# atakan-topaloglu/stable-virtual-camera

Hardware: AMD Instinct MI355X
Metric: denoising steps/sec, 1.3B Seva @ 21x576x576 views (higher is better)
Workload: dtype f16; 1 GPU; Seva 1.3B (1,263,968,004 params, random-init), one 21-view window per GPU, 576x576 px (latent 72x72), CFG batch 42, Euler-EDM step, MultiviewCFG(1.2) cfg 2.0; novel_views_per_sec = value x (T - 1 input view) / 50 steps per window; views=21, latent=72, windows=1

## Files before the change

### include/seva_hip.h

```cpp
#ifndef SEVA_HIP_H
#define SEVA_HIP_H

#include <stdint.h>

#ifdef __cplusplus
extern "C" {
#endif

typedef void* seva_stream_t;

#define SEVA_OK 0
#define SEVA_ERR_ARG (-1)
#define SEVA_ERR_LAUNCH (-2)
#define SEVA_ERR_UNSUPPORTED (-3)

const char* seva_last_error(void);
int seva_abi_version(void);
const char* seva_target_arch(void);

typedef struct seva_gemm_desc {
  const void* a;
  const void* w;
  const float* bias;
  const float* row_add;
// ... 14 lines not shown
  void* out_f8;
  int64_t ldo8;
  float* ch_stats;
  float* splitk_ws;
  int64_t splitk_ws_bytes;
  const void* a2;
  int64_t lda2;
  int64_t K2;
  int64_t alg_K;
} seva_gemm_desc;
int seva_gemm_f16(const seva_gemm_desc* d, seva_stream_t stream);
int seva_gemm_fp8(const seva_gemm_desc* d, seva_stream_t stream);

typedef struct seva_ff_desc {
  const void* a;
  const void* w1;
  const float* b1;
  const void* w2;
  const float* b2;
  const float* residual;
  float* out_f32;
  void* out_f16;
  int64_t M, lda, ldr, ldo32, ldo16;
  int32_t C;
  const float* ln_x;
  const float* ln_gamma;
  const float* ln_beta;
  int64_t ldx;
  float ln_eps;
  const void* w1_exp;
  const void* w2_exp;
} seva_ff_desc;
int seva_ff_fused_f16(const seva_ff_desc* d, seva_stream_t stream);
int seva_ff_fused_fp8(const seva_ff_desc* d, seva_stream_t stream);

typedef struct seva_attn_desc {
  const void* q;
  const void* k;
  const void* v;
  void* out;
  int64_t q_sb0, q_sb1, q_sl;
  int64_t k_sb0, k_sb1, k_sl;
  int64_t o_sb0, o_sb1, o_sl;
  int32_t nb0, nb1;
  int32_t heads;
  int32_t lq, lk;
  float scale;
  int32_t q_prescaled;
  float* split_ws;
  int64_t split_ws_bytes;
} seva_attn_desc;
int seva_attention_f16(const seva_attn_desc* d, seva_stream_t stream);

int seva_attn_v_fp8_size(int32_t batch, int32_t heads, int32_t lk, int64_t* v8_bytes, int64_t* scale_bytes);
int seva_attn_quant_v_fp8(const seva_attn_desc* d, void* v8, uint8_t* v8_scale, seva_stream_t stream);
int seva_attention_pv8(const seva_attn_desc* d, const void* v8, const uint8_t* v8_scale, seva_stream_t stream);

#define SEVA_GN_WORKSPACE_SLABS 1024
typedef struct seva_groupnorm_desc {
  const float* x1;
  const float* x2;
  const float* gamma;
  const float* beta;
  const float* dense;
  const float* dense_w;
  const float* dense_b;
  void* out_f16;
  float* workspace;
  int32_t n, hw, c1, c2, groups, dense_c, silu;
  float eps;
  void* raw_f16;
  void* out_f8;
  int64_t ld_out_f8;
  const float* stats1;
  const float* stats2;
  int32_t split_out_f16;
  int32_t split_raw_f16;
} seva_groupnorm_desc;
int seva_groupnorm_f16(const seva_groupnorm_desc* d, seva_stream_t stream);

int seva_layernorm_f16(const float* x, const float* gamma, const float* beta, void* out_f16,
                       int64_t rows, int32_t c, float eps, seva_stream_t stream);
int seva_layernorm_fp8(const float* x, const float* gamma, const float* beta, void* out_f8, int64_t rows,
                       int32_t c, float eps, int64_t ld_out ,
                       seva_stream_t stream);

int seva_softmax_rows_f16(const float* x, int64_t ldx, void* out_f16, int64_t ldo, int64_t rows,
                          int32_t cols, int32_t cols_pad, float scale, seva_stream_t stream);

int seva_nchw_to_nhwc_f16(const float* x1, int32_t c1, const float* x2, int32_t c2,
                          const float* scale, void* out_f16, int32_t n, int32_t hw, int32_t cpad,
                          seva_stream_t stream);
int seva_nchw_to_nhwc_f16_split(const float* x1, int32_t c1, const float* x2, int32_t c2,
                                const float* scale, void* out_f16, int32_t n, int32_t hw, int32_t cpad,
                                seva_stream_t stream);
int seva_nhwc_to_nchw_f32(const float* x, int64_t ld, float* out, int32_t n, int32_t c,
                          int32_t hw, seva_stream_t stream);
int seva_cast_concat_f16(const float* x1, int32_t c1, const float* x2, int32_t c2, void* out_f16,
                         int64_t rows, seva_stream_t stream);
int seva_bilinear_to_nhwc_f32(const float* src, float* out, int32_t n, int32_t c, int32_t sh,
                              int32_t sw, int32_t oh, int32_t ow, seva_stream_t stream);
int seva_timestep_embedding_f16(const int64_t* t, const float* freqs, void* out_f16, int32_t n,
                                int32_t dim, seva_stream_t stream);
int seva_silu_f16(const float* x, void* out_f16, int64_t count, seva_stream_t stream);
int seva_add_f32(const float* a, const float* b, float* out, int64_t count, seva_stream_t stream);

// ... 51 lines not shown
```

### stable-virtual-camera_amd/seva/_engine.py

```python

from __future__ import annotations

import math
import os

import torch

from . import _native, ops
from ._arch import Layout
from ._native import SevaNativeError, require_cuda

F16, F32, U8 = torch.float16, torch.float32, torch.uint8
QK_SCALE_LOG2E = 0.125 * 1.4426950408889634
CIN_PAD = 64


def _pad128(k: int) -> int:
    return 128 * ((k + 127) // 128)


def pack_conv3x3(w: torch.Tensor, cin_pad: int | None = None) -> torch.Tensor:
    cout, cin = w.shape[:2]
    cin_pad = cin_pad or cin
    out = torch.zeros((cout, 3, 3, cin_pad), dtype=F16, device=w.device)
# ... 38 lines not shown

    def nbytes(self) -> int:
        return sum(t.numel() * t.element_size() for t in self.bufs.values())


class SevaEngine:
    @staticmethod
    def _resolve_device(model) -> torch.device:
        params = [p for p in model.parameters()]
        if not params or params[0].device.type != "cuda":
            raise SevaNativeError(
                "Seva.forward runs only on an AMD GPU: move the module to a cuda device first "
                "(there is no CPU fallback)."
            )
        from . import _native

        _native.load()
        return params[0].device

    def __init__(self, model, precision: str | None = None, attention: str | None = None, ff: str | None = None):
        import os as _os

        self.device = self._resolve_device(model)
        self.precision = precision or _os.environ.get("SEVA_PRECISION", "f16")
        if self.precision not in ("f16", "fp8"):
            raise ValueError(f"unknown precision {self.precision!r} (f16 | fp8)")
        self.fp8 = self.precision == "fp8"
        if attention is None:
            attention = "fp8" if self.fp8 and _os.environ.get("SEVA_FP8_ATTENTION", "0") == "1" else "f16"
        if attention not in ("f16", "fp8"):
            raise ValueError(f"unknown attention {attention!r} (f16 | fp8)")
        if attention == "fp8" and not self.fp8:
            raise ValueError('attention="fp8" needs precision "fp8" (the f16 parity mode stays pure)')
        self.attention = attention
        self.pv8 = attention == "fp8"
        self.fp8_pad = _os.environ.get("SEVA_FP8_PAD", "0") == "1"
        self.ff_fused = _os.environ.get("SEVA_FF_FUSED", "1") != "0"
        if ff is None:
            ff = "fp8" if self.fp8 and _os.environ.get("SEVA_FP8_FF", "0") == "1" else "f16"
        if ff not in ("f16", "fp8"):
            raise ValueError(f"unknown ff {ff!r} (f16 | fp8)")
        if ff == "fp8" and not self.fp8:
            raise ValueError('ff="fp8" needs precision "fp8" (the f16 parity mode stays pure)')
        self.ff = ff
        self.ff8 = ff == "fp8"
        self.gn_fused_stats = int(_os.environ.get("SEVA_GN_FUSED_STATS", "1"))
        self._stats: dict = {}
        self.conv_splitk = _os.environ.get("SEVA_CONV_SPLITK", "1") != "0"
        self.attn_split = _os.environ.get("SEVA_ATTN_SPLIT_KV", "1") != "0"
        self.attn_split_max = max(2, min(4, int(_os.environ.get("SEVA_ATTN_SPLIT", "2"))))
        self.fold_skip = _os.environ.get("SEVA_FOLD_SKIP", "0") != "0" and not self.fp8
        sp = _os.environ.get("SEVA_SPLIT_PRECISION", "stem,head,skip_deep")
        self.split = {t for t in sp.split(",") if t} if not self.fp8 else set()
        self.p = model.params
        self.layout: Layout = model._layout
        self.arena = _Arena(self.device)
        self._pack(model)
        import os

        self.use_graph = os.environ.get("SEVA_HIPGRAPH", "1") != "0"
        self._graphs: dict = {}
        self.slice_frames = int(os.environ.get("SEVA_SLICE_FRAMES", "0"))
        self.slice_min_bytes = int(float(os.environ.get("SEVA_SLICE_MIN_MB", "96")) * (1 << 20))
        self.slice_attn = os.environ.get("SEVA_SLICE_ATTN", "0") == "1"

    def _ff_fused_fp8(self, c: int) -> bool:
        return self.ff8 and self.ff_fused and c in ops.FF_FUSED_CHANNELS and c % 128 != 0

    def _split_skip(self, cout: int) -> bool:
        return "skip" in self.split or ("skip_deep" in self.split and cout >= 2 * self.p.model_channels)

    def _pack(self, model) -> None:
        sd = {k: v.detach() for k, v in model.state_dict().items()}
        dev = self.device
        W: dict[str, torch.Tensor] = {}

        def f16(k):
            return sd[k].to(device=dev, dtype=F16).contiguous()

        def f32(k):
            return sd[k].to(device=dev, dtype=F32).contiguous()

        mc = self.p.model_channels
        half = mc // 2
        W["freqs"] = torch.exp(
            -math.log(10000) * torch.arange(start=0, end=half, dtype=torch.float32) / half
        ).to(dev)
        for k in ("time_embed.0", "time_embed.2"):
            W[k + ".w"], W[k + ".b"] = f16(k + ".weight"), f32(k + ".bias")

        emb_w, emb_b, ctx_w, ctx_b = [], [], [], []
        self.emb_off: dict[str, int] = {}
        self.ctx_off: dict[str, int] = {}
        emb_total = ctx_total = 0

        def q8(name, w):
            if not (self.fp8 and w.shape[0] % 16 == 0 and w.shape[0] > 32):
                return
            k = w.shape[1]
            kp = _pad128(k)
            if kp != k and (not self.fp8_pad or kp * 4 > k * 5):
                return
            if kp != k:
                w = torch.cat([w, w.new_zeros((w.shape[0], kp - k))], 1)
            W[name + "8"], W[name + "8e"] = ops.quantize_weight_fp8(w)

        def pack_attn_self(pfx):
            W[pfx + ".qkv"] = torch.cat(
                [f16(pfx + ".to_q.weight"), f16(pfx + ".to_k.weight"), f16(pfx + ".to_v.weight")], 0
            ).contiguous()
            q8(pfx + ".qkv", torch.cat([f32(pfx + ".to_q.weight"), f32(pfx + ".to_k.weight"), f32(pfx + ".to_v.weight")], 0))
            W[pfx + ".out.w"], W[pfx + ".out.b"] = f16(pfx + ".to_out.0.weight"), f32(pfx + ".to_out.0.bias")

        def pack_attn_cross(pfx):
            nonlocal ctx_total
            wv, wo = f32(pfx + ".to_v.weight"), f32(pfx + ".to_out.0.weight")
            ctx_w.append((wo.double() @ wv.double()).to(F16))
            ctx_b.append(f32(pfx + ".to_out.0.bias"))
            self.ctx_off[pfx] = ctx_total
            ctx_total += wo.shape[0]
            W[pfx + ".q"] = f16(pfx + ".to_q.weight")
            W[pfx + ".kv"] = torch.cat([f16(pfx + ".to_k.weight"), f16(pfx + ".to_v.weight")], 0).contiguous()
            W[pfx + ".out.w"], W[pfx + ".out.b"] = f16(pfx + ".to_out.0.weight"), f32(pfx + ".to_out.0.bias")

        def pack_ff(pfx):
            wi, bi = interleave_geglu(f16(pfx + ".net.0.proj.weight"), f32(pfx + ".net.0.proj.bias"))
            W[pfx + ".w1"], W[pfx + ".b1"] = wi, bi
            W[pfx + ".w2"], W[pfx + ".b2"] = f16(pfx + ".net.2.weight"), f32(pfx + ".net.2.bias")
            if self._ff_fused_fp8(wi.shape[1]):
                W[pfx + ".w1f8"], W[pfx + ".w1f8e"], W[pfx + ".w2f8"], W[pfx + ".w2f8e"] = ops.pack_ff_fp8(
                    interleave_geglu(f32(pfx + ".net.0.proj.weight"), f32(pfx + ".net.0.proj.bias"))[0], f32(pfx + ".net.2.weight"))
            elif self.fp8:
                q8(pfx + ".w1", interleave_geglu(f32(pfx + ".net.0.proj.weight"), f32(pfx + ".net.0.proj.bias"))[0])
                if pfx + ".w18" in W:
                    q8(pfx + ".w2", f32(pfx + ".net.2.weight"))

        def pack_ln(pfx):
            W[pfx + ".g"], W[pfx + ".b"] = f32(pfx + ".weight"), f32(pfx + ".bias")

        for spec in self.layout.all_specs():
            pfx = spec.prefix
            if spec.kind == "conv":
                wc = f32(pfx + ".weight")
                if "stem" in self.split and 2 * spec.cin <= CIN_PAD:
                    wc = torch.cat([wc, wc], 1)
                W[pfx + ".w"] = pack_conv3x3(wc, CIN_PAD * ((wc.shape[1] + CIN_PAD - 1) // CIN_PAD))
                W[pfx + ".b"] = f32(pfx + ".bias")
            elif spec.kind == "res":
                assert spec.cin % 64 == 0 and spec.cout % 64 == 0, "channel counts must be multiples of 64"
                pack_ln(pfx + ".in_layers.0")
                pack_ln(pfx + ".out_layers.0")
                W[pfx + ".conv1.w"] = pack_conv3x3(f32(pfx + ".in_layers.2.weight"))
                W[pfx + ".conv1.b"] = f32(pfx + ".in_layers.2.bias")
                W[pfx + ".conv2.w"] = pack_conv3x3(f32(pfx + ".out_layers.3.weight"))
                W[pfx + ".conv2.b"] = f32(pfx + ".out_layers.3.bias")
                if self.fp8:
                    for tag, key, ch in (("conv1", "in_layers.2", spec.cin), ("conv2", "out_layers.3", spec.cout)):
                        cp = _pad128(ch)
                        if cp == ch or (self.fp8_pad and cp * 4 <= ch * 5):
                            q8(f"{pfx}.{tag}.w", pack_conv3x3(f32(f"{pfx}.{key}.weight"), cp).float())
                W[pfx + ".dense.w"] = f32(pfx + ".dense_emb_layers.0.weight").reshape(2 * spec.cin, -1).contiguous()
                W[pfx + ".dense.b"] = f32(pfx + ".dense_emb_layers.0.bias")
                emb_w.append(f16(pfx + ".emb_layers.1.weight"))
                emb_b.append(f32(pfx + ".emb_layers.1.bias"))
                self.emb_off[pfx] = emb_total
# ... 140 lines not shown
        else:
            ops.conv3x3(a16.view(n, h, w, cin), W[pfx + ".conv1.w"], bias=W[pfx + ".conv1.b"],
                        row_add=emb_all[:, off:], rows_per_group=hw, ld_row_add=self.emb_total, out_f32=hmid, ch_stats=st_mid,
                        splitk_ws=self._sk(n * hw, hw, cout))
        b16 = None if f8_2 else self._buf("gn16", (n, hw, cout), F16)
        b8 = self._buf("gn8", (n, hw, cout8), U8, zero=True) if f8_2 else None
        ops.groupnorm(hmid, None, W[pfx + ".out_layers.0.g"], W[pfx + ".out_layers.0.b"], b16, self.gn_ws,
                      eps=1e-5, silu=True, out_f8=b8, stats1=st_mid)
        fold = cin != cout and self.fold_skip and not f8_2 and (hw > 128 or not self.conv_splitk)
        if fold:
            res = None
        elif cin != cout:
            res = self._buf("skip32", (n * hw, cout), F32)
            ops.gemm(xs16, W[pfx + ".skip.w"], bias=W[pfx + ".skip.b"], out_f32=res, alg_k=cin)
        else:
            assert x2 is None
            res = x1
        out = self._buf("out:" + pfx, (n, hw, cout), F32)
        st_out = self._stats_buf("out:" + pfx, n * hw, hw, cout)
        if fold:
            ops.conv3x3(b16.view(n, h, w, cout), W[pfx + ".conv2.wf"], bias=W[pfx + ".conv2.bf"], a2=xs16, out_f32=out,
                        ch_stats=st_out)
        elif f8_2:
            ops.conv3x3(b8.view(n, h, w, cout8), W[pfx + ".conv2.w8"], w_exp=W[pfx + ".conv2.w8e"], bias=W[pfx + ".conv2.b"],
                        residual=res, out_f32=out, ch_stats=st_out)
        else:
            ops.conv3x3(b16.view(n, h, w, cout), W[pfx + ".conv2.w"], bias=W[pfx + ".conv2.b"],
                        residual=res, out_f32=out, ch_stats=st_out, splitk_ws=self._sk(n * hw, hw, cout))
        self._produced(out, st_out)
        return out

    def _self_attention(self, x32, ln_pfx, at_pfx, rows, c, heads, *, regime, n, hw, T, residual,
                        row_add, rpg, ldra, out_f32):
        W = self.W
        c3 = 3 * c
        if regime == "frame" and self.slice_attn and self._slice_rows(rows, c, hw) < rows:
            step = self._slice_rows(rows, c, hw)
            a_buf = self._buf("ln16", (step, c), F16)
            qkv_buf = self._buf("qkv", (step, c3), F16)
            att_buf = self._buf("att", (step, c), F16)
            for r0 in range(0, rows, step):
                r1 = min(r0 + step, rows)
                nr, f0, nf = r1 - r0, r0 // hw, (r1 - r0) // hw
                a, qkv, att = a_buf[:nr], qkv_buf[:nr], att_buf[:nr]
                ops.layernorm(x32[r0:r1], W[ln_pfx + ".g"], W[ln_pfx + ".b"], a)
                ops.gemm(a, W[at_pfx + ".qkv"], out_f16=qkv, col_scale=QK_SCALE_LOG2E, col_scale_n=c)
                ops.attention(qkv[:, :c], qkv[:, c:2 * c], qkv[:, 2 * c:], att, nb0=nf, nb1=1, heads=heads, lq=hw, lk=hw,
                              q_strides=(hw * c3, 0, c3), k_strides=(hw * c3, 0, c3), o_strides=(hw * c, 0, c),
                              q_prescaled=True)
                ops.gemm(att, W[at_pfx + ".out.w"], bias=W[at_pfx + ".out.b"], residual=residual[r0:r1],
                         row_add=None if row_add is None else row_add[f0:], rows_per_group=rpg, ld_row_add=ldra,
                         out_f32=out_f32[r0:r1])
            return
        qkv = self._buf("qkv", (rows, 3 * c), F16)
        if at_pfx + ".qkv8" in W:
            a8 = self._ln(x32, ln_pfx, rows, c, fp8=True)
            ops.gemm(a8, W[at_pfx + ".qkv8"], w_exp=W[at_pfx + ".qkv8e"], out_f16=qkv, col_scale=QK_SCALE_LOG2E, col_scale_n=c)
        else:
            a = self._ln(x32, ln_pfx, rows, c)
            ops.gemm(a, W[at_pfx + ".qkv"], out_f16=qkv, col_scale=QK_SCALE_LOG2E, col_scale_n=c)
        att = self._buf("att", (rows, c), F16)
        q, k, v = qkv[:, :c], qkv[:, c:2 * c], qkv[:, 2 * c:]
        if regime == "frame":
            self._attention_long(q, k, v, att, nb0=n, heads=heads, L=hw, q_strides=(hw * c3, 0, c3),
                                 k_strides=(hw * c3, 0, c3), o_strides=(hw * c, 0, c), split_ws=None)
        elif regime == "joint":
            sws = None
            if self.attn_split and T * hw >= ops.ATTN_SPLIT_MIN_LK:
                sws = self._buf("attn_split", (ops.attention_split_workspace_numel(n // T, heads, T * hw, self.attn_split_max),), F32)
            self._attention_long(q, k, v, att, nb0=n // T, heads=heads, L=T * hw, q_strides=(T * hw * c3, 0, c3),
                                 k_strides=(T * hw * c3, 0, c3), o_strides=(T * hw * c, 0, c), split_ws=sws)
        else:
            ops.attention(q, k, v, att, nb0=n // T, nb1=hw, heads=heads, lq=T, lk=T,
                          q_strides=(T * hw * c3, c3, hw * c3), k_strides=(T * hw * c3, c3, hw * c3),
                          o_strides=(T * hw * c, c, hw * c), q_prescaled=True)
        ops.gemm(att, W[at_pfx + ".out.w"], bias=W[at_pfx + ".out.b"], residual=residual,
                 row_add=row_add, rows_per_group=rpg, ld_row_add=ldra, out_f32=out_f32)

    def _attention_long(self, q, k, v, att, *, nb0, heads, L, q_strides, k_strides, o_strides, split_ws):
        if self.pv8 and L >= ops.PV8_MIN_LQ:
            ws = self._buf("v_fp8", (ops.v_fp8_workspace_numel(nb0, heads, L),), U8)
            ops.quantize_v_fp8(v, ws, nb0=nb0, nb1=1, heads=heads, lk=L, k_strides=k_strides)
            ops.attention_pv8(q, k, ws, att, nb0=nb0, nb1=1, heads=heads, lq=L, lk=L, q_strides=q_strides,
                              k_strides=k_strides, o_strides=o_strides, split_ws=split_ws)
            return
        ops.attention(q, k, v, att, nb0=nb0, nb1=1, heads=heads, lq=L, lk=L, q_strides=q_strides, k_strides=k_strides,
                      o_strides=o_strides, q_prescaled=True, split_ws=split_ws)

    def _cross_attention_general(self, x32, ln_pfx, at_pfx, rows, c, heads, ctx16, lc, *, nb0, nb1,
                                 lq, q_strides, o_strides, ctx_batch_stride, out_f32):
        W = self.W
        a = self._ln(x32, ln_pfx, rows, c)
        q = self._buf("xq", (rows, c), F16)
        ops.gemm(a, W[at_pfx + ".q"], out_f16=q)
        kv = self._buf("xkv", (ctx16.shape[0], 2 * c), F16)
        ops.gemm(ctx16, W[at_pfx + ".kv"], out_f16=kv)
        att = self._buf("att", (rows, c), F16)
        ops.attention(q, kv[:, :c], kv[:, c:], att, nb0=nb0, nb1=nb1, heads=heads, lq=lq, lk=lc,
                      q_strides=q_strides, k_strides=(ctx_batch_stride * 2 * c, 0, 2 * c),
                      o_strides=o_strides)
        ops.gemm(att, W[at_pfx + ".out.w"], bias=W[at_pfx + ".out.b"], residual=x32, out_f32=out_f32)

    def _transformer(self, spec, x, n, h, w, T, ctxvec, ctx16, lc):
        W, pfx, hw, c, heads = self.W, spec.prefix, h * w, spec.channels, spec.heads
        rows = n * hw
        g16 = self._buf("gn16", (n, hw, c), F16)
# ... 236 lines not shown
```

### stable-virtual-camera_amd/seva/_native.py

```python

from __future__ import annotations

import ctypes as C
import os
from ctypes import POINTER, c_char_p, c_double, c_float, c_int, c_int32, c_int64, c_void_p

import torch

_HERE = os.path.dirname(os.path.abspath(__file__))
LIB_PATH = os.environ.get("SEVA_HIP_LIB") or os.path.join(os.path.dirname(_HERE), "libseva_hip.so")
ABI_VERSION = 12
PROF_CLASSES = 5
PROF_NAMES = ("gemm", "conv", "attention", "norm", "elementwise")


class SevaNativeError(RuntimeError):
    pass


class GemmDesc(C.Structure):
    _fields_ = [
        ("a", c_void_p), ("w", c_void_p), ("bias", c_void_p), ("row_add", c_void_p),
        ("residual", c_void_p), ("out_f32", c_void_p), ("out_f16", c_void_p),
        ("M", c_int64), ("N", c_int64), ("K", c_int64),
        ("lda", c_int64), ("ldr", c_int64), ("ldo32", c_int64), ("ldo16", c_int64),
        ("rows_per_group", c_int64), ("ld_row_add", c_int64),
        ("mode", c_int32), ("epilogue", c_int32),
        ("n", c_int32), ("ih", c_int32), ("iw", c_int32), ("cin", c_int32),
        ("oh", c_int32), ("ow", c_int32), ("stride", c_int32), ("upsample", c_int32),
        ("col_scale", c_float), ("col_scale_n", c_int32), ("pad_br_only", c_int32),
        ("w_exp", c_void_p), ("out_f8", c_void_p), ("ldo8", c_int64),
        ("ch_stats", c_void_p), ("splitk_ws", c_void_p), ("splitk_ws_bytes", c_int64),
        ("a2", c_void_p), ("lda2", c_int64), ("K2", c_int64),
        ("alg_K", c_int64),
    ]


class FfDesc(C.Structure):
    _fields_ = [
        ("a", c_void_p), ("w1", c_void_p), ("b1", c_void_p), ("w2", c_void_p), ("b2", c_void_p),
        ("residual", c_void_p), ("out_f32", c_void_p), ("out_f16", c_void_p),
        ("M", c_int64), ("lda", c_int64), ("ldr", c_int64), ("ldo32", c_int64), ("ldo16", c_int64),
        ("C", c_int32),
        ("ln_x", c_void_p), ("ln_gamma", c_void_p), ("ln_beta", c_void_p), ("ldx", c_int64), ("ln_eps", c_float),
        ("w1_exp", c_void_p), ("w2_exp", c_void_p),
    ]


class AttnDesc(C.Structure):
    _fields_ = [
        ("q", c_void_p), ("k", c_void_p), ("v", c_void_p), ("out", c_void_p),
        ("q_sb0", c_int64), ("q_sb1", c_int64), ("q_sl", c_int64),
        ("k_sb0", c_int64), ("k_sb1", c_int64), ("k_sl", c_int64),
        ("o_sb0", c_int64), ("o_sb1", c_int64), ("o_sl", c_int64),
        ("nb0", c_int32), ("nb1", c_int32), ("heads", c_int32),
        ("lq", c_int32), ("lk", c_int32), ("scale", c_float), ("q_prescaled", c_int32),
        ("split_ws", c_void_p), ("split_ws_bytes", c_int64),
    ]


class GroupNormDesc(C.Structure):
    _fields_ = [
        ("x1", c_void_p), ("x2", c_void_p), ("gamma", c_void_p), ("beta", c_void_p),
        ("dense", c_void_p), ("dense_w", c_void_p), ("dense_b", c_void_p),
        ("out_f16", c_void_p), ("workspace", c_void_p),
        ("n", c_int32), ("hw", c_int32), ("c1", c_int32), ("c2", c_int32),
        ("groups", c_int32), ("dense_c", c_int32), ("silu", c_int32), ("eps", c_float),
        ("raw_f16", c_void_p), ("out_f8", c_void_p), ("ld_out_f8", c_int64),
        ("stats1", c_void_p), ("stats2", c_void_p),
        ("split_out_f16", c_int32), ("split_raw_f16", c_int32),
    ]


SYMBOLS = {
    "seva_last_error": (c_char_p, []),
    "seva_abi_version": (c_int, []),
    "seva_target_arch": (c_char_p, []),
    "seva_gemm_f16": (c_int, [POINTER(GemmDesc), c_void_p]),
    "seva_gemm_fp8": (c_int, [POINTER(GemmDesc), c_void_p]),
    "seva_ff_fused_f16": (c_int, [POINTER(FfDesc), c_void_p]),
    "seva_ff_fused_fp8": (c_int, [POINTER(FfDesc), c_void_p]),
    "seva_attention_f16": (c_int, [POINTER(AttnDesc), c_void_p]),
    "seva_attn_v_fp8_size": (c_int, [c_int32, c_int32, c_int32, POINTER(c_int64), POINTER(c_int64)]),
    "seva_attn_quant_v_fp8": (c_int, [POINTER(AttnDesc), c_void_p, c_void_p, c_void_p]),
    "seva_attention_pv8": (c_int, [POINTER(AttnDesc), c_void_p, c_void_p, c_void_p]),
    "seva_groupnorm_f16": (c_int, [POINTER(GroupNormDesc), c_void_p]),
    "seva_layernorm_f16": (c_int, [c_void_p, c_void_p, c_void_p, c_void_p, c_int64, c_int32, c_float, c_void_p]),
    "seva_layernorm_fp8": (c_int, [c_void_p, c_void_p, c_void_p, c_void_p, c_int64, c_int32, c_float, c_int64, c_void_p]),
    "seva_layernorm_f32": (c_int, [c_void_p, c_void_p, c_void_p, c_void_p, c_int64, c_int32, c_float, c_void_p]),
    "seva_clip_preprocess_f16": (c_int, [c_void_p, c_void_p, c_int32, c_int32, c_int32, c_int32, c_int32, c_int32,
                                         c_void_p, c_void_p, c_int32, c_void_p]),
    "seva_attention_small_f16": (c_int, [c_void_p, c_void_p, c_void_p, c_void_p, c_int64, c_int64, c_int64, c_int64,
                                         c_int64, c_int64, c_int32, c_int32, c_int32, c_int32, c_float, c_void_p]),
    "seva_softmax_rows_f16": (c_int, [c_void_p, c_int64, c_void_p, c_int64, c_int64, c_int32, c_int32, c_float, c_void_p]),
    "seva_nchw_to_nhwc_f16": (c_int, [c_void_p, c_int32, c_void_p, c_int32, c_void_p, c_void_p, c_int32, c_int32, c_int32, c_void_p]),
    "seva_nchw_to_nhwc_f16_split": (c_int, [c_void_p, c_int32, c_void_p, c_int32, c_void_p, c_void_p, c_int32, c_int32, c_int32, c_void_p]),
    "seva_nhwc_to_nchw_f32": (c_int, [c_void_p, c_int64, c_void_p, c_int32, c_int32, c_int32, c_void_p]),
    "seva_cast_concat_f16": (c_int, [c_void_p, c_int32, c_void_p, c_int32, c_void_p, c_int64, c_void_p]),
    "seva_bilinear_to_nhwc_f32": (c_int, [c_void_p, c_void_p, c_int32, c_int32, c_int32, c_int32, c_int32, c_int32, c_void_p]),
    "seva_timestep_embedding_f16": (c_int, [c_void_p, c_void_p, c_void_p, c_int32, c_int32, c_void_p]),
    "seva_silu_f16": (c_int, [c_void_p, c_void_p, c_int64, c_void_p]),
    "seva_add_f32": (c_int, [c_void_p, c_void_p, c_void_p, c_int64, c_void_p]),
    "seva_replace_blend_f32": (c_int, [c_void_p, c_void_p, c_void_p, c_int32, c_int32, c_int32, c_void_p]),
    "seva_denoiser_combine_f32": (c_int, [c_void_p, c_void_p, c_void_p, c_void_p, c_void_p, c_int32, c_int64, c_void_p]),
    "seva_add_noise_f32": (c_int, [c_void_p, c_void_p, c_void_p, c_void_p, c_int32, c_int64, c_void_p]),
    "seva_cfg_euler_f32": (c_int, [c_void_p, c_void_p, c_void_p, c_void_p, c_void_p, c_void_p, c_int32, c_int64, c_void_p]),
    "seva_cfg_combine_f32": (c_int, [c_void_p, c_void_p, c_void_p, c_int32, c_int64, c_void_p]),
    "seva_euler_step_f32": (c_int, [c_void_p, c_void_p, c_void_p, c_void_p, c_void_p, c_int32, c_int64, c_void_p]),
    "seva_to_d_f32": (c_int, [c_void_p, c_void_p, c_void_p, c_void_p, c_int32, c_int64, c_void_p]),
    "seva_scale_rows_f32": (c_int, [c_void_p, c_void_p, c_void_p, c_int32, c_int64, c_void_p]),
    "seva_plucker_f32": (c_int, [c_void_p, c_void_p, c_void_p, c_int32, c_int32, c_int32, c_void_p]),
    "seva_cond_concat_f32": (c_int, [c_void_p, c_void_p, c_void_p, c_void_p, c_int32, c_int32, c_int32, c_void_p]),
    "seva_set_knob": (c_int, [c_char_p, c_int32]),
    "seva_get_knob": (c_int, [c_char_p, POINTER(c_int32)]),
    "seva_graph_begin": (c_int, [c_void_p]),
    "seva_graph_end": (c_int, [c_void_p, POINTER(c_void_p)]),
    "seva_graph_launch": (c_int, [c_void_p, c_void_p]),
    "seva_graph_destroy": (c_int, [c_void_p]),
    "seva_prof_enable": (c_int, [c_int]),
    "seva_prof_collect": (c_int, [POINTER(c_double), POINTER(c_int64), POINTER(c_double), POINTER(c_double)]),
}

_lib = None

_EAGER_DEPTH = 0


class eager_network:
    def __enter__(self):
        global _EAGER_DEPTH
        _EAGER_DEPTH += 1

    def __exit__(self, *exc):
        global _EAGER_DEPTH
        _EAGER_DEPTH -= 1
# ... 57 lines not shown
```

### stable-virtual-camera_amd/seva/ops.py

```python

from __future__ import annotations

import ctypes as C

import torch

from . import _native as nv
from ._native import AttnDesc, GemmDesc, GroupNormDesc, check, ptr, require_cuda, stream_ptr

F16, F32 = torch.float16, torch.float32
U8 = torch.uint8


def _lib():
    return nv.load()


def gemm(
    a: torch.Tensor,
    w: torch.Tensor,
    *,
    bias: torch.Tensor | None = None,
    row_add: torch.Tensor | None = None,
    rows_per_group: int = 0,
    ld_row_add: int = 0,
    residual: torch.Tensor | None = None,
    out_f32: torch.Tensor | None = None,
    out_f16: torch.Tensor | None = None,
    geglu: bool = False,
    col_scale: float = 1.0,
    col_scale_n: int = 0,
    w_exp: torch.Tensor | None = None,
    out_f8: torch.Tensor | None = None,
    ch_stats: torch.Tensor | None = None,
    splitk_ws: torch.Tensor | None = None,
    alg_k: int = 0,
) -> None:
    fp8 = w_exp is not None
    require_cuda(a, w)
    assert a.dim() == 2 and w.dim() == 2 and a.dtype == w.dtype == (U8 if fp8 else F16)
    M, K = a.shape
    N = w.shape[0]
    d = GemmDesc()
    d.a, d.w = ptr(a), w.data_ptr()
    d.bias, d.row_add, d.residual = ptr(bias), ptr(row_add), ptr(residual)
    d.out_f32, d.out_f16 = ptr(out_f32), ptr(out_f16)
    d.M, d.N, d.K = M, N, K
    d.alg_K = alg_k
    d.lda = a.stride(0)
    d.ldr = residual.stride(0) if residual is not None else 0
    d.ldo32 = out_f32.stride(0) if out_f32 is not None else 0
    d.ldo16 = out_f16.stride(0) if out_f16 is not None else 0
    d.rows_per_group, d.ld_row_add = rows_per_group, ld_row_add
    d.mode, d.epilogue = 0, 1 if geglu else 0
    d.col_scale, d.col_scale_n = col_scale, col_scale_n
    d.ch_stats = _stats_ptr(ch_stats, M, N, out_f32)
    if splitk_ws is not None and not fp8:
        assert splitk_ws.dtype == F32 and splitk_ws.is_contiguous()
        d.splitk_ws, d.splitk_ws_bytes = splitk_ws.data_ptr(), splitk_ws.numel() * 4
        _register_handoff_ws(splitk_ws)
    if fp8:
# ... 198 lines not shown
                      ch_stats: torch.Tensor | None = None, alg_k: int = 0) -> None:
    require_cuda(x, w4)
    assert x.dtype == w4.dtype == F16 and x.dim() == 4 and x.is_contiguous() and w4.is_contiguous()
    n, ih, iw, cin = x.shape
    assert w4.dim() == 3 and w4.shape[0] == 4 and w4.shape[2] == 4 * cin, "w4: [4, cout, 4 * cin]"
    if ch_stats is not None:
        raise ValueError("conv3x3_up_phases emits no GroupNorm statistics (ch_stats must be None)")
    if out_f32 is None:
        raise ValueError("conv3x3_up_phases needs out_f32")
    oh, ow = 2 * ih, 2 * iw
    d = GemmDesc()
    d.a, d.w, d.bias, d.out_f32 = x.data_ptr(), w4.data_ptr(), ptr(bias), out_f32.data_ptr()
    d.M, d.N, d.K = n * oh * ow, w4.shape[1], 4 * cin
    d.alg_K = alg_k
    d.lda, d.ldo32 = cin, out_f32.stride(-2)
    d.mode, d.epilogue = 1, 0
    d.n, d.ih, d.iw, d.cin, d.oh, d.ow = n, ih, iw, cin, oh, ow
    d.stride, d.upsample = 1, 2
    check(_lib().seva_gemm_f16(C.byref(d), stream_ptr(x.device)), "seva_gemm_f16(conv, upsample phases)")


def attention(
    q: torch.Tensor,
    k: torch.Tensor,
    v: torch.Tensor,
    out: torch.Tensor,
    *,
    nb0: int,
    nb1: int,
    heads: int,
    lq: int,
    lk: int,
    q_strides: tuple[int, int, int],
    k_strides: tuple[int, int, int],
    o_strides: tuple[int, int, int],
    scale: float = 0.125,
    q_prescaled: bool = False,
    split_ws: torch.Tensor | None = None,
) -> None:
    require_cuda(q, k, v, out)
    d = AttnDesc()
    d.q, d.k, d.v, d.out = q.data_ptr(), k.data_ptr(), v.data_ptr(), out.data_ptr()
    d.q_sb0, d.q_sb1, d.q_sl = q_strides
    d.k_sb0, d.k_sb1, d.k_sl = k_strides
    d.o_sb0, d.o_sb1, d.o_sl = o_strides
    d.nb0, d.nb1, d.heads, d.lq, d.lk, d.scale = nb0, nb1, heads, lq, lk, scale
    d.q_prescaled = 1 if q_prescaled else 0
    if split_ws is not None:
        assert split_ws.dtype == F32 and split_ws.is_contiguous()
        d.split_ws, d.split_ws_bytes = split_ws.data_ptr(), split_ws.numel() * 4
    check(_lib().seva_attention_f16(C.byref(d), stream_ptr(q.device)), "seva_attention_f16")


ATTN_SPLIT_MIN_LK = 6144


def attention_split_workspace_numel(batch: int, heads: int, lq: int, nsplit: int = 2) -> int:
    return nsplit * batch * heads * lq * 66


PV8_MIN_LQ = 2048


def _v_fp8_parts(batch: int, heads: int, lk: int) -> tuple[int, int]:
    v8, sc = C.c_int64(), C.c_int64()
    check(_lib().seva_attn_v_fp8_size(batch, heads, lk, C.byref(v8), C.byref(sc)), "seva_attn_v_fp8_size")
    return v8.value, sc.value


def v_fp8_workspace_numel(batch: int, heads: int, lk: int) -> int:
    v8, sc = _v_fp8_parts(batch, heads, lk)
    return v8 + sc


def _v_fp8_ptrs(ws: torch.Tensor, batch: int, heads: int, lk: int) -> tuple[int, int]:
    v8, sc = _v_fp8_parts(batch, heads, lk)
    assert ws.dtype == U8 and ws.is_contiguous() and ws.numel() >= v8 + sc, "v_fp8 workspace too small"
    return ws.data_ptr(), ws.data_ptr() + v8


def _attn_desc(q, k, v, out, nb0, nb1, heads, lq, lk, q_strides, k_strides, o_strides, split_ws) -> AttnDesc:
    d = AttnDesc()
    d.q, d.k, d.v, d.out = ptr(q), ptr(k), ptr(v), ptr(out)
    d.q_sb0, d.q_sb1, d.q_sl = q_strides
    d.k_sb0, d.k_sb1, d.k_sl = k_strides
    d.o_sb0, d.o_sb1, d.o_sl = o_strides
    d.nb0, d.nb1, d.heads, d.lq, d.lk = nb0, nb1, heads, lq, lk
    d.q_prescaled = 1
    if split_ws is not None:
        assert split_ws.dtype == F32 and split_ws.is_contiguous()
        d.split_ws, d.split_ws_bytes = split_ws.data_ptr(), split_ws.numel() * 4
    return d


def quantize_v_fp8(v: torch.Tensor, ws: torch.Tensor, *, nb0: int, nb1: int, heads: int, lk: int,
                   k_strides: tuple[int, int, int]) -> None:
    require_cuda(v, ws)
    v8, sc = _v_fp8_ptrs(ws, nb0 * nb1, heads, lk)
    d = _attn_desc(None, None, v, None, nb0, nb1, heads, lk, lk, (0, 0, 0), k_strides, (0, 0, 0), None)
    check(_lib().seva_attn_quant_v_fp8(C.byref(d), v8, sc, stream_ptr(v.device)), "seva_attn_quant_v_fp8")


def attention_pv8(q: torch.Tensor, k: torch.Tensor, ws: torch.Tensor, out: torch.Tensor, *, nb0: int, nb1: int, heads: int,
                  lq: int, lk: int, q_strides: tuple[int, int, int], k_strides: tuple[int, int, int],
                  o_strides: tuple[int, int, int], split_ws: torch.Tensor | None = None) -> None:
    require_cuda(q, k, ws, out)
# ... 321 lines not shown
```

Baseline: 11.21 denoising steps/s.

## Fuse temporal-attention QKV projection and attention into one kernel

```diff
diff --git a/include/seva_hip.h b/include/seva_hip.h
--- a/include/seva_hip.h
+++ b/include/seva_hip.h
@@ -90,6 +90,17 @@
 } seva_attn_desc;
 int seva_attention_f16(const seva_attn_desc* d, seva_stream_t stream);
 
+typedef struct seva_tmix_desc {
+  const void* a;
+  const void* w;
+  void* out;
+  int64_t a_sb0, a_sb1, a_sl;
+  int64_t o_sb0, o_sb1, o_sl;
+  int32_t scenes, hw, T, C;
+  float col_scale;
+} seva_tmix_desc;
+int seva_tmix_attention_f16(const seva_tmix_desc* d, seva_stream_t stream);
+
 int seva_attn_v_fp8_size(int32_t batch, int32_t heads, int32_t lk, int64_t* v8_bytes, int64_t* scale_bytes);
 int seva_attn_quant_v_fp8(const seva_attn_desc* d, void* v8, uint8_t* v8_scale, seva_stream_t stream);
 int seva_attention_pv8(const seva_attn_desc* d, const void* v8, const uint8_t* v8_scale, seva_stream_t stream);
diff --git a/stable-virtual-camera_amd/csrc/tmix_fused.hip b/stable-virtual-camera_amd/csrc/tmix_fused.hip
--- /dev/null
+++ b/stable-virtual-camera_amd/csrc/tmix_fused.hip
@@ -0,0 +1,322 @@
+#include "gemm_common.h"
+
+namespace {
+
+constexpr int BK = 64;
+constexpr int BM = 128;
+constexpr int BN = 192;
+constexpr int NJ = BN / 16, MI = 2, KS_A = 10;
+constexpr int B_BYTES = BN * 128, B_PASSES = BN / 32;
+constexpr int PART_BYTES = BM * 128;
+constexpr int LDS_BYTES = 2 * B_BYTES;
+static_assert(3 * PART_BYTES == LDS_BYTES, "the q/k/v exchange tile is exactly the weight ring");
+
+struct TmixArgs {
+  const half_t* a;
+  const half_t* w;
+  half_t* out;
+  int64_t a_sb0, a_sb1, a_sl;
+  int64_t o_sb0, o_sb1, o_sl;
+  int32_t K, T, hw, heads, P, tiles_per_scene;
+  float col_scale;
+};
+
+typedef short short8_t __attribute__((ext_vector_type(8)));
+
+template <int N>
+__device__ __forceinline__ void wait_vm() {
+  asm volatile("s_waitcnt vmcnt(%0)" ::"n"(N) : "memory");
+}
+__device__ __forceinline__ void barrier_raw() {
+  asm volatile("s_waitcnt lgkmcnt(0)" ::: "memory");
+  __builtin_amdgcn_s_barrier();
+  asm volatile("" ::: "memory");
+}
+__device__ __forceinline__ void glds16_sbase(const void* sbase, unsigned voff, unsigned lds_wave_base) {
+  unsigned keep;
+  asm volatile(
+      "s_mov_b32 %0, m0\n\ts_mov_b32 m0, %3\n\ts_nop 0\n\tglobal_load_lds_dwordx4 %1, %2\n\ts_mov_b32 m0, %0"
+      : "=&s"(keep)
+      : "v"(voff), "s"(sbase), "s"(lds_wave_base)
+      : "memory");
+}
+__device__ __forceinline__ half8_t tr_read_pair(const char* a0, const char* a1) {
+  short4_t lo = __builtin_amdgcn_ds_read_tr16_b64_v4i16((__attribute__((address_space(3))) short4_t*)a0);
+  short4_t hi = __builtin_amdgcn_ds_read_tr16_b64_v4i16((__attribute__((address_space(3))) short4_t*)a1);
+  short8_t s = __builtin_shufflevector(lo, hi, 0, 1, 2, 3, 4, 5, 6, 7);
+  return __builtin_bit_cast(half8_t, s);
+}
+__device__ __forceinline__ int v_chunk_swz(int row, int chunk) { return chunk ^ (((row >> 1) & 1) << 2); }
+__device__ __forceinline__ int k_chunk_swz(int row, int chunk) { return chunk ^ ((row >> 1) & 7); }
+__device__ __forceinline__ float half_wave_max(float v) {
+  float a = v, b = v;
+  asm volatile("s_nop 1\n\tv_permlane32_swap_b32 %0, %1" : "+v"(a), "+v"(b));
+  return fmaxf(a, b);
+}
+
+__global__ __launch_bounds__(256, 2) void tmix_qkv_attn_kernel(TmixArgs p) {
+  extern __shared__ __attribute__((aligned(16))) char smem[];
+
+  const int lane = threadIdx.x & 63;
+  const int wave = __builtin_amdgcn_readfirstlane(threadIdx.x >> 6);
+  const int fr = lane & 15, fg = lane >> 4;
+  const int nk = p.K / BK;
+  const int T = p.T;
+
+  const int scene = blockIdx.x / p.tiles_per_scene;
+  const int pix0 = (blockIdx.x - scene * p.tiles_per_scene) * p.P;
+  const int npix = p.hw - pix0 < p.P ? p.hw - pix0 : p.P;
+
+  half8_t areg[MI][KS_A];
+#pragma unroll
+  for (int i = 0; i < MI; ++i) {
+    int r = wave * 32 + 16 * i + fr;
+    if (r >= p.P * T) r = p.P * T - 1;
+    int pp = r / T;
+    const int t = r - pp * T;
+    if (pp >= npix) pp = npix - 1;
+    const half_t* ap = p.a + scene * p.a_sb0 + (int64_t)(pix0 + pp) * p.a_sb1 + t * p.a_sl + 8 * fg;
+#pragma unroll
+    for (int ks = 0; ks < KS_A; ++ks) {
+      const int kk = 32 * ks < p.K ? 32 * ks : 0;
+      areg[i][ks] = *(const half8_t*)(ap + kk);
+    }
+  }
+#pragma unroll
+  for (int i = 0; i < MI; ++i)
+#pragma unroll
+    for (int ks = 0; ks < KS_A; ++ks) asm volatile("" : "+v"(areg[i][ks]));
+
+  auto b_key = [](int row) { return ((row >> 1) & 1) | (((row >> 3) & 3) << 1); };
+  auto lane_now = [&]() {
+    int l = lane;
+    asm volatile("" : "+v"(l));
+    return l;
+  };
+  const unsigned lds_base_u32 = __builtin_amdgcn_readfirstlane(lds_addr_u32(smem));
+  auto stage = [&](int head, int buf, int kt) {
+    const unsigned lb = lds_base_u32 + buf * B_BYTES + wave * (BN / 4) * 128;
+    const int l = lane_now(), sr = l >> 3, sp = l & 7;
+    const unsigned wl = (unsigned)((wave * (BN / 4) + sr) * p.K) * 2u;
+    const unsigned lp = (unsigned)(sp ^ ((sr >> 1) & 1)) << 4;
+#pragma unroll
+    for (int i = 0; i < B_PASSES; ++i) {
+      const half_t* const sbase = p.w + ((head * BN + 8 * i) * p.K + kt * BK);
+      const unsigned key_hi = (unsigned)((wave * (BN / 32) + i) & 3) << 5;
+      glds16_sbase(sbase, wl + (lp ^ key_hi), lb + i * 1024);
+    }
+  };
+  int b_off[2];
+#pragma unroll
+  for (int s = 0; s < 2; ++s) {
+    const int rb = 8 * (fr >> 2) + (fr & 3);
+    b_off[s] = rb * 128 + (((4 * s + fg) ^ b_key(rb)) << 4);
+  }
+  auto b_frag_off = [&](int s, int j) { return b_off[s] + (32 * (j >> 1) + 4 * (j & 1)) * 128; };
+
+  char* const img_q = smem;
+  char* const img_k = smem + PART_BYTES;
+  char* const img_v = smem + 2 * PART_BYTES;
+
+  stage(0, 0, 0);
+  if (nk > 1) stage(0, 1, 1);
+  for (int head = 0; head < p.heads; ++head) {
+    f32x4 acc[MI][NJ];
+#pragma unroll
+    for (int i = 0; i < MI; ++i)
+#pragma unroll
+      for (int j = 0; j < NJ; ++j) acc[i][j] = f32x4{0.f, 0.f, 0.f, 0.f};
+
+    if (nk > 1) wait_vm<B_PASSES>();
+    else wait_vm<0>();
+    barrier_raw();
+    auto ktile = [&](int kt) {
+      const int cur = kt & 1;
+      if (kt >= 1 && kt + 1 < nk) stage(head, cur ^ 1, kt + 1);
+      const char* const tb = smem + cur * B_BYTES;
+#pragma unroll
+      for (int s2 = 0; s2 < 2; ++s2) {
+#pragma unroll
+        for (int jh = 0; jh < NJ; jh += NJ / 2) {
+          half8_t bfr[NJ / 2];
+#pragma unroll
+          for (int j = 0; j < NJ / 2; ++j) bfr[j] = *(const half8_t*)(tb + b_frag_off(s2, jh + j));
+#pragma unroll
+          for (int i = 0; i < MI; ++i)
+#pragma unroll
+            for (int j = 0; j < NJ / 2; ++j)
+              acc[i][jh + j] = __builtin_amdgcn_mfma_f32_16x16x32_f16(bfr[j], areg[i][2 * kt + s2], acc[i][jh + j], 0, 0, 0);
+        }
+      }
+      if (kt + 1 < nk) wait_vm<0>();
+      barrier_raw();
+    };
+#pragma unroll
+    for (int kt = 0; kt < KS_A / 2; ++kt)
+      if (kt < nk) ktile(kt);
+
+    const int lx = lane_now(), fr = lx & 15, fg = lx >> 4;
+#pragma unroll
+    for (int i = 0; i < MI; ++i) {
+      const int r = wave * 32 + 16 * i + fr;
+#pragma unroll
+      for (int j = 0; j < NJ; j += 2) {
+        const int part = j >> 2;
+        const int chunk = 4 * ((j >> 1) & 1) + fg;
+        f32x4 v0 = acc[i][j], v1 = acc[i][j + 1];
+        if (part == 0) {
+          v0 *= p.col_scale;
+          v1 *= p.col_scale;
+        }
+        const half8_t h = {(half_t)v0[0], (half_t)v0[1], (half_t)v0[2], (half_t)v0[3],
+                           (half_t)v1[0], (half_t)v1[1], (half_t)v1[2], (half_t)v1[3]};
+        const int pc = part == 2 ? v_chunk_swz(r, chunk) : k_chunk_swz(r, chunk);
+        *(half8_t*)(smem + part * PART_BYTES + r * 128 + (pc << 4)) = h;
+      }
+    }
+    barrier_raw();
+
+    const int la = lane_now(), qi = la & 31, hh = la >> 5, q4 = (la & 15) >> 2, p4 = la & 3;
+    for (int pp = wave; pp < npix; pp += 4) {
+      const int rb0 = pp * T;
+      const int qrow = rb0 + (qi < T ? qi : T - 1);
+      half8_t qf[4];
+#pragma unroll
+      for (int s = 0; s < 4; ++s) qf[s] = *(const half8_t*)(img_q + qrow * 128 + (k_chunk_swz(qrow, 2 * s + hh) << 4));
+      f32x16 sc;
+      {
+        const int krow = rb0 + qi < BM ? rb0 + qi : BM - 1;
+#pragma unroll
+        for (int s = 0; s < 4; ++s) {
+          const half8_t kf = *(const half8_t*)(img_k + krow * 128 + (k_chunk_swz(krow, 2 * s + hh) << 4));
+          if (s == 0) {
+            f32x16 c0;
+#pragma unroll
+            for (int r = 0; r < 16; ++r) c0[r] = 0.f;
+            sc = __builtin_amdgcn_mfma_f32_32x32x16_f16(kf, qf[s], c0, 0, 0, 0);
+          } else {
+            sc = __builtin_amdgcn_mfma_f32_32x32x16_f16(kf, qf[s], sc, 0, 0, 0);
+          }
+        }
+      }
+#pragma unroll
+      for (int r = 0; r < 16; ++r) {
+        const int key = (r & 3) + 8 * (r >> 2) + 4 * hh;
+        if (key >= T) sc[r] = -1e30f;
+      }
+      float mx = -1e30f;
+      {
+        float mk = sc[0];
+#pragma unroll
+        for (int r = 1; r < 16; ++r) mk = fmaxf(mk, sc[r]);
+        mx = fmaxf(mx, mk);
+        mx = half_wave_max(mx);
+      }
+      const float delta = mx;
+#pragma unroll
+      for (int r = 0; r < 16; ++r) sc[r] -= delta;
+      typedef __fp16 fp16x2_t __attribute__((ext_vector_type(2)));
+      const fp16x2_t ones2 = {(__fp16)1.0f, (__fp16)1.0f};
+      float lsum4[4] = {0.f, 0.f, 0.f, 0.f};
+      half8_t pf[2];
+#pragma unroll
+      for (int s2 = 0; s2 < 2; ++s2) {
+        fp16x2_t pk[4];
+#pragma unroll
+        for (int j = 0; j < 4; ++j) {
+          const float e0 = __builtin_amdgcn_exp2f(sc[8 * s2 + 2 * j]);
+          const float e1 = __builtin_amdgcn_exp2f(sc[8 * s2 + 2 * j + 1]);
+          pk[j] = __builtin_amdgcn_cvt_pkrtz(e0, e1);
+          lsum4[j] = __builtin_amdgcn_fdot2(pk[j], ones2, lsum4[j], false);
+        }
+        pf[s2] = __builtin_bit_cast(half8_t, pk);
+      }
+      const float l_run = (lsum4[0] + lsum4[1]) + (lsum4[2] + lsum4[3]);
+      f32x16 acc_o[2];
+#pragma unroll
+      for (int d = 0; d < 2; ++d)
+#pragma unroll
+        for (int r = 0; r < 16; ++r) acc_o[d][r] = 0.f;
+#pragma unroll
+      for (int db = 0; db < 2; ++db) {
+#pragma unroll
+        for (int s2 = 0; s2 < 2; ++s2) {
+          const int r0 = 16 * s2 + 4 * hh;
+          const int colbyte = (32 * db + 16 * ((la >> 4) & 1) + 4 * p4) * 2;
+          const int ch = colbyte >> 4, within = colbyte & 15;
+          int ra = rb0 + r0 + q4, rb = rb0 + r0 + 8 + q4;
+          if (ra >= BM) ra = BM - 1;
+          if (rb >= BM) rb = BM - 1;
+          const half8_t vf = tr_read_pair(img_v + ra * 128 + (v_chunk_swz(ra, ch) << 4) + within,
+                                          img_v + rb * 128 + (v_chunk_swz(rb, ch) << 4) + within);
+          acc_o[db] = __builtin_amdgcn_mfma_f32_32x32x16_f16(vf, pf[s2], acc_o[db], 0, 0, 0);
+        }
+      }
+      const float l_tot = l_run + __shfl_xor(l_run, 32, 64);
+      const float inv = 1.0f / l_tot;
+      if (qi < T) {
+        const int orow = rb0 + qi;
+#pragma unroll
+        for (int db = 0; db < 2; ++db)
+#pragma unroll
+          for (int t = 0; t < 4; ++t) {
+            half4_t h;
+#pragma unroll
+            for (int r = 0; r < 4; ++r) h[r] = (half_t)(acc_o[db][4 * t + r] * inv);
+            const int d0 = 32 * db + 8 * t + 4 * hh;
+            const int chunk = d0 >> 3, piece = (d0 >> 2) & 1;
+            *(half4_t*)(img_q + orow * 128 + ((chunk ^ (orow & 7)) << 4) + (piece << 3)) = h;
+          }
+      }
+      __builtin_amdgcn_s_waitcnt(0xc07f);
+      __builtin_amdgcn_wave_barrier();
+      half_t* const obase = p.out + scene * p.o_sb0 + (int64_t)(pix0 + pp) * p.o_sb1 + head * 64;
+#pragma unroll
+      for (int i = 0; i < 4; ++i) {
+        const int t = 8 * i + (la >> 3), pchunk = la & 7;
+        if (t < T) {
+          const int orow = rb0 + t;
+          const uint4 v = *(const uint4*)(img_q + orow * 128 + (pchunk << 4));
+          const int lchunk = pchunk ^ (orow & 7);
+          *(uint4*)(obase + (int64_t)t * p.o_sl + lchunk * 8) = v;
+        }
+      }
+    }
+    barrier_raw();
+    if (head + 1 < p.heads) {
+      stage(head + 1, 0, 0);
+      if (nk > 1) stage(head + 1, 1, 1);
+    }
+  }
+}
+
+}
+
+extern "C" int seva_tmix_attention_f16(const seva_tmix_desc* d, seva_stream_t stream) {
+  SEVA_REQUIRE(d != nullptr, "tmix: null desc");
+  SEVA_REQUIRE(d->a && d->w && d->out, "tmix: null pointer");
+  SEVA_REQUIRE(d->scenes > 0 && d->hw > 0, "tmix: empty problem scenes=%d hw=%d", d->scenes, d->hw);
+  SEVA_REQUIRE(d->T >= 1 && d->T <= 32, "tmix: T=%d outside [1, 32]", d->T);
+  SEVA_REQUIRE(d->C >= 64 && d->C <= 320 && d->C % 64 == 0, "tmix: C=%d must be a multiple of 64, at most 320", d->C);
+  SEVA_REQUIRE(((uintptr_t)d->a | (uintptr_t)d->w | (uintptr_t)d->out) % 16 == 0, "tmix: pointers must be 16-byte aligned");
+  SEVA_REQUIRE((d->a_sb0 | d->a_sb1 | d->a_sl | d->o_sb0 | d->o_sb1 | d->o_sl) % 8 == 0, "tmix: strides must be multiples of 8 elements");
+  TmixArgs a{};
+  a.a = (const half_t*)d->a;
+  a.w = (const half_t*)d->w;
+  a.out = (half_t*)d->out;
+  a.a_sb0 = d->a_sb0; a.a_sb1 = d->a_sb1; a.a_sl = d->a_sl;
+  a.o_sb0 = d->o_sb0; a.o_sb1 = d->o_sb1; a.o_sl = d->o_sl;
+  a.K = d->C; a.T = d->T; a.hw = d->hw; a.heads = d->C / 64;
+  a.P = BM / d->T;
+  a.tiles_per_scene = (d->hw + a.P - 1) / a.P;
+  a.col_scale = d->col_scale;
+  const int64_t nb = (int64_t)d->scenes * a.tiles_per_scene;
+  SEVA_REQUIRE(nb <= 0x7fffffff, "tmix: bad grid %lld", (long long)nb);
+  hipStream_t s = (hipStream_t)stream;
+  const double rows = (double)d->scenes * d->hw * d->T;
+  const double flops = 2.0 * rows * 3.0 * d->C * d->C + 4.0 * rows * d->T * d->C;
+  const double alg_bytes = 2.0 * (2.0 * rows * d->C + 3.0 * d->C * d->C);
+  SevaProfScope prof(0, flops, s, alg_bytes);
+  hipLaunchKernelGGL(tmix_qkv_attn_kernel, dim3((unsigned)nb), dim3(256), LDS_BYTES, s, a);
+  return seva_check_launch("tmix_qkv_attn_kernel");
+}
diff --git a/stable-virtual-camera_amd/seva/_engine.py b/stable-virtual-camera_amd/seva/_engine.py
--- a/stable-virtual-camera_amd/seva/_engine.py
+++ b/stable-virtual-camera_amd/seva/_engine.py
@@ -114,6 +114,8 @@
         self.fold_skip = _os.environ.get("SEVA_FOLD_SKIP", "0") != "0" and not self.fp8
         sp = _os.environ.get("SEVA_SPLIT_PRECISION", "stem,head,skip_deep")
         self.split = {t for t in sp.split(",") if t} if not self.fp8 else set()
+        self.tmix_fused = (not self.fp8 and _os.environ.get("SEVA_TMIX_FUSED", "1") != "0"
+                           and getattr(ops, "tmix_attention", None) is not None)
         self.p = model.params
         self.layout: Layout = model._layout
         self.arena = _Arena(self.device)
@@ -173,6 +175,8 @@
             ).contiguous()
             q8(pfx + ".qkv", torch.cat([f32(pfx + ".to_q.weight"), f32(pfx + ".to_k.weight"), f32(pfx + ".to_v.weight")], 0))
             W[pfx + ".out.w"], W[pfx + ".out.b"] = f16(pfx + ".to_out.0.weight"), f32(pfx + ".to_out.0.bias")
+            if ".time_mix_blocks." in pfx and self.tmix_fused and W[pfx + ".qkv"].shape[1] <= ops.TMIX_FUSED_MAX_C:
+                W[pfx + ".qkv_heads"] = ops.pack_qkv_heads(W[pfx + ".qkv"])
 
         def pack_attn_cross(pfx):
             nonlocal ctx_total
@@ -419,6 +423,15 @@
                          row_add=None if row_add is None else row_add[f0:], rows_per_group=rpg, ld_row_add=ldra,
                          out_f32=out_f32[r0:r1])
             return
+        if regime == "temporal" and at_pfx + ".qkv_heads" in W and T <= ops.TMIX_FUSED_MAX_T:
+            a = self._ln(x32, ln_pfx, rows, c)
+            att = self._buf("att", (rows, c), F16)
+            ops.tmix_attention(a, W[at_pfx + ".qkv_heads"], att, scenes=n // T, hw=hw, T=T,
+                               a_strides=(T * hw * a.stride(0), a.stride(0), hw * a.stride(0)),
+                               o_strides=(T * hw * c, c, hw * c), col_scale=QK_SCALE_LOG2E)
+            ops.gemm(att, W[at_pfx + ".out.w"], bias=W[at_pfx + ".out.b"], residual=residual,
+                     row_add=row_add, rows_per_group=rpg, ld_row_add=ldra, out_f32=out_f32)
+            return
         qkv = self._buf("qkv", (rows, 3 * c), F16)
         if at_pfx + ".qkv8" in W:
             a8 = self._ln(x32, ln_pfx, rows, c, fp8=True)
diff --git a/stable-virtual-camera_amd/seva/_native.py b/stable-virtual-camera_amd/seva/_native.py
--- a/stable-virtual-camera_amd/seva/_native.py
+++ b/stable-virtual-camera_amd/seva/_native.py
@@ -59,6 +59,16 @@
     ]
 
 
+class TmixDesc(C.Structure):
+    _fields_ = [
+        ("a", c_void_p), ("w", c_void_p), ("out", c_void_p),
+        ("a_sb0", c_int64), ("a_sb1", c_int64), ("a_sl", c_int64),
+        ("o_sb0", c_int64), ("o_sb1", c_int64), ("o_sl", c_int64),
+        ("scenes", c_int32), ("hw", c_int32), ("T", c_int32), ("C", c_int32),
+        ("col_scale", c_float),
+    ]
+
+
 class GroupNormDesc(C.Structure):
     _fields_ = [
         ("x1", c_void_p), ("x2", c_void_p), ("gamma", c_void_p), ("beta", c_void_p),
@@ -81,6 +91,7 @@
     "seva_ff_fused_f16": (c_int, [POINTER(FfDesc), c_void_p]),
     "seva_ff_fused_fp8": (c_int, [POINTER(FfDesc), c_void_p]),
     "seva_attention_f16": (c_int, [POINTER(AttnDesc), c_void_p]),
+    "seva_tmix_attention_f16": (c_int, [POINTER(TmixDesc), c_void_p]),
     "seva_attn_v_fp8_size": (c_int, [c_int32, c_int32, c_int32, POINTER(c_int64), POINTER(c_int64)]),
     "seva_attn_quant_v_fp8": (c_int, [POINTER(AttnDesc), c_void_p, c_void_p, c_void_p]),
     "seva_attention_pv8": (c_int, [POINTER(AttnDesc), c_void_p, c_void_p, c_void_p]),
diff --git a/stable-virtual-camera_amd/seva/ops.py b/stable-virtual-camera_amd/seva/ops.py
--- a/stable-virtual-camera_amd/seva/ops.py
+++ b/stable-virtual-camera_amd/seva/ops.py
@@ -6,7 +6,7 @@
 import torch
 
 from . import _native as nv
-from ._native import AttnDesc, GemmDesc, GroupNormDesc, check, ptr, require_cuda, stream_ptr
+from ._native import AttnDesc, GemmDesc, GroupNormDesc, TmixDesc, check, ptr, require_cuda, stream_ptr
 
 F16, F32 = torch.float16, torch.float32
 U8 = torch.uint8
@@ -311,6 +311,31 @@
     check(_lib().seva_attention_f16(C.byref(d), stream_ptr(q.device)), "seva_attention_f16")
 
 
+TMIX_FUSED_MAX_C = 320
+TMIX_FUSED_MAX_T = 32
+
+
+def pack_qkv_heads(wqkv: torch.Tensor) -> torch.Tensor:
+    c3, c = wqkv.shape
+    assert c3 == 3 * c and c % 64 == 0
+    return wqkv.view(3, c // 64, 64, c).permute(1, 0, 2, 3).reshape(c3, c).contiguous()
+
+
+def tmix_attention(a: torch.Tensor, w_heads: torch.Tensor, out: torch.Tensor, *, scenes: int, hw: int, T: int,
+                   a_strides: tuple[int, int, int], o_strides: tuple[int, int, int], col_scale: float) -> None:
+    require_cuda(a, w_heads, out)
+    assert a.dtype == w_heads.dtype == out.dtype == F16 and w_heads.dim() == 2 and w_heads.is_contiguous()
+    c = w_heads.shape[1]
+    assert w_heads.shape[0] == 3 * c and a.stride(-1) == 1 and out.stride(-1) == 1
+    d = TmixDesc()
+    d.a, d.w, d.out = a.data_ptr(), w_heads.data_ptr(), out.data_ptr()
+    d.a_sb0, d.a_sb1, d.a_sl = a_strides
+    d.o_sb0, d.o_sb1, d.o_sl = o_strides
+    d.scenes, d.hw, d.T, d.C = scenes, hw, T, c
+    d.col_scale = col_scale
+    check(_lib().seva_tmix_attention_f16(C.byref(d), stream_ptr(a.device)), "seva_tmix_attention_f16")
+
+
 ATTN_SPLIT_MIN_LK = 6144
 
 
```

Result: no change. 11.30 denoising steps/s (median of 6 runs) (+0.8%).
